# omkhairate/MetalPathtracer

Hardware: AMD Instinct MI355X
Metric: Mrays/s at 1920x1080x256spp on scene.xml (higher is better)
Workload: dtype f32; 1 GPU; scene.xml 1920x1080 x 256 spp per step, depth 8 (181 steps timed); prims=4971, bvh_nodes=2289, bvh_builder=device, rng=philox4x32-10 (pixel,sample,bounce), pipeline=wave-local wavefront, reference-order walk, parallelism=8x8-tile interleave over 1 rank(s), rays=161154900585

## Files before the change

metalpathtracer_amd/csrc/mpt_kernels.h:

```cpp
#pragma once
#include <hip/hip_runtime.h>
#include <stdint.h>

#include "mpt_device.h"
#include "mpt_wl_lean.h"
#include "mpt_lean_entry.h"
#include "mpt_lean_tiles.h"

#ifndef MPT_MIN_WAVES
#define MPT_MIN_WAVES 8
#endif

struct QueueDev {
    float4* od;
    float4* dt;
    float4* tl;
    uint2* ia;
};

struct PassDesc {
    uint32_t in_count[MPT_NSHARD];
    uint32_t item_prefix[MPT_NSHARD + 1];
    uint32_t n_items;
    uint32_t regen_base;
// ... 353 lines not shown
__device__ __forceinline__ void announce_resident(const PassParams& pp) {
    if (pp.launch_id == 0u) return;
    const uint32_t before = atomicAdd(&pp.ctr[MPT_CTR_STARTED], 1u);
    if (before == 0u) __hip_atomic_store(&pp.desc->t_first, (unsigned long long)__builtin_amdgcn_s_memrealtime(), __ATOMIC_RELAXED, __HIP_MEMORY_SCOPE_AGENT);
    if (before + 1u == gridDim.x)
        __hip_atomic_store((uint32_t*)pp.host_done + MPT_HOST_RESIDENT, pp.launch_id, __ATOMIC_RELAXED, __HIP_MEMORY_SCOPE_SYSTEM);
}

__device__ __forceinline__ void note_wave_exit(const PassParams& pp) {
    if (pp.launch_id == 0u || (threadIdx.x & 63u) != 0u) return;
    const uint32_t before = atomicAdd(&pp.ctr[MPT_CTR_EXITED], 1u);
    if (before + 1u == gridDim.x * (blockDim.x >> 6)) {
        const unsigned long long t0 = __hip_atomic_load(&pp.desc->t_first, __ATOMIC_RELAXED, __HIP_MEMORY_SCOPE_AGENT);
        atomicAdd(&pp.desc->trace_ticks, (unsigned long long)__builtin_amdgcn_s_memrealtime() - t0);
    }
}

__global__ void k_begin_pass(PassDesc* d, uint32_t* ctr, uint32_t total_paths, uint32_t slots_items,
                             volatile uint32_t* host_done, int path_cursors) {
    if (threadIdx.x != 0 || blockIdx.x != 0) return;
    ctr[MPT_CTR_STARTED] = 0u;
    ctr[MPT_CTR_EXITED] = 0u;
    if (path_cursors) {
        d->total_paths = total_paths;
        for (uint32_t g = 0; g < MPT_NGROUP; ++g) ctr[MPT_CTR_CURSOR(g)] = 0u;
        return;
    }
    for (uint32_t s = 0; s < MPT_NSHARD; ++s) ctr[MPT_CTR_OUT(s)] = 0;
    d->next_path = 0;
    d->total_paths = total_paths;
    d->slots_items = slots_items;
    d->iterations = 0;
    advance_desc(d, ctr, host_done);
}

__global__ void k_advance(PassDesc* d, uint32_t* ctr, volatile uint32_t* host_done) {
    if (threadIdx.x != 0 || blockIdx.x != 0) return;
    advance_desc(d, ctr, host_done);
}

template <bool COUNT, bool ALL_LDS>
__global__ __launch_bounds__(1024, MPT_MIN_WAVES) void k_megakernel(PassParams pp) {
    extern __shared__ float4 lds_nodes[];
    stage_nodes(pp.scene, lds_nodes);
    const uint32_t lane = threadIdx.x & 63u;
    const uint32_t total_paths = pp.desc->total_paths;
    const uint32_t waves_per_block = blockDim.x >> 6;
    uint32_t n_rays = 0, n_paths = 0;
    WorkCount wc = {};
    for (uint32_t chunk = blockIdx.x * waves_per_block + (threadIdx.x >> 6); chunk * 64u < total_paths;
         chunk += gridDim.x * waves_per_block) {
        PathState ps;
        PathRngDev g;
        ps.path = chunk * 64u + lane;
        uint32_t px, py, s;
        if (!path_to_pixel(pp, ps.path, px, py, s)) continue;
        gen_primary(pp, px, py, pp.sample_begin + s, ps, g);
        n_paths++;
        bool alive = true;
        while (alive) {
            float t;
            int prim;
            closest_hit<COUNT, ALL_LDS>(pp.scene, (LdsNodes)lds_nodes, ps.o, ps.d, t, prim, wc);
            n_rays++;
            alive = shade_bounce(pp.scene, (LdsNodes)lds_nodes, pp.sp, g, ps, t, prim);
        }
        pp.slots[ps.path] = make_float4(clamp01(ps.L.x), clamp01(ps.L.y), clamp01(ps.L.z), clamp01(ps.La));
    }
    flush_stats<COUNT>(pp.desc, n_rays, n_paths, wc);
}

typedef float v4f_nt __attribute__((ext_vector_type(4)));
__device__ __forceinline__ void store_slot(float4* slots, uint32_t path, float r, float g, float b, float a) {
    v4f_nt v = {r, g, b, a};
    __builtin_nontemporal_store(v, (v4f_nt*)(slots + path));
}
__device__ __forceinline__ float4 load_slot(const float4* slots, uint32_t idx) {
    v4f_nt v = __builtin_nontemporal_load((const v4f_nt*)(slots + idx));
    return make_float4(v.x, v.y, v.z, v.w);
}

__device__ __forceinline__ uint32_t wave_rank(unsigned long long m) {
    return __builtin_amdgcn_mbcnt_hi((uint32_t)(m >> 32), __builtin_amdgcn_mbcnt_lo((uint32_t)m, 0u));
}

#ifndef MPT_WL_LEVELS
#define MPT_WL_LEVELS 2u
#endif
#define MPT_WL_RING 512u
#define MPT_LDS_MATS_N 32u
#define MPT_LDS_CFG_F4 16u
static_assert(CFG_F4_END <= MPT_LDS_CFG_F4, "configuration block too small");
__host__ __device__ __forceinline__ uint32_t mpt_lds_cfg_off_f4(uint32_t lds_mat_off) { return lds_mat_off + 2u * MPT_LDS_MATS_N; }
__host__ __device__ __forceinline__ uint32_t mpt_lds_image_end_f4(uint32_t lds_mat_off) { return mpt_lds_cfg_off_f4(lds_mat_off) + MPT_LDS_CFG_F4; }
#define MPT_WL_BLOCK 1024u
#define MPT_WL_TILE_ELIDED 0x40000000u
static_assert((MPT_WL_TILE_ELIDED & (MPT_LEAN_TILES_SKIP | MPT_LEAN_TILES_MASK_BITS)) == 0u, "the elision mark shares a bit with the class word");
#define MPT_WL_NO_BUDGET 0x7FFFFFFFu

__device__ __forceinline__ void cfg_stage_common(float4* blk, const PassParams& pp, float rW, float rH, uint32_t wl_block, uint32_t wl_min, uint32_t wl_div) {
    blk[CFG_F4_CAM] = make_float4(pp.cam.x, pp.cam.y, pp.cam.z, pp.W);
    blk[CFG_F4_FIRST] = make_float4(pp.first.x, pp.first.y, pp.first.z, pp.H);
    blk[CFG_F4_VU] = make_float4(pp.vu.x, pp.vu.y, pp.vu.z, rW);
    blk[CFG_F4_VV] = make_float4(pp.vv.x, pp.vv.y, pp.vv.z, rH);
    uint32_t* w = (uint32_t*)(blk + CFG_F4_WORDS);
    w[CFG_W_CLAIM_BLOCK] = wl_block;
    w[CFG_W_CLAIM_MIN] = wl_min;
    w[CFG_W_CLAIM_DIV] = wl_div * (((uint32_t)(gridDim.x * (blockDim.x >> 6)) + MPT_NGROUP - 1u) / MPT_NGROUP);
    w[CFG_W_RANK_TILES] = pp.desc->total_paths / (pp.S * 64u);
}
__device__ __forceinline__ CamView cfg_cam_view(LdsNodes blk) {
    const v4f c0 = blk[CFG_F4_CAM], c1 = blk[CFG_F4_FIRST], c2 = blk[CFG_F4_VU], c3 = blk[CFG_F4_VV];
    CamView cv;
    cv.cam = f3(c0.x, c0.y, c0.z);
    cv.first = f3(c1.x, c1.y, c1.z);
    cv.vu = f3(c2.x, c2.y, c2.z);
    cv.vv = f3(c3.x, c3.y, c3.z);
    cv.W = c0.w;
    cv.H = c1.w;
    cv.rW = c2.w;
    cv.rH = c3.w;
    return cv;
}
__device__ __forceinline__ bool claim_paths(const PassParams& pp, LdsWords cfg, uint32_t lane, uint32_t& grp, uint32_t& seen, uint32_t& k, uint32_t& blk,
                                            uint32_t& rend) {
    bool got = false;
    k = 0, blk = 0, rend = 0;
    if (lane == 0) {
        const uint32_t c_block = cfg[CFG_W_CLAIM_BLOCK], c_min = cfg[CFG_W_CLAIM_MIN], c_div = cfg[CFG_W_CLAIM_DIV], c_tiles = cfg[CFG_W_RANK_TILES];
        for (uint32_t t = 0; t < MPT_NGROUP && !got; ++t) {
            const uint32_t re = range_paths(c_tiles, pp.S, grp);
            const uint32_t left = seen < re ? re - seen : 0u;
            blk = (left / c_div) & ~63u;
            blk = blk < c_min ? c_min : (blk > c_block ? c_block : blk);
            if (t > 0u) blk = c_min;
            k = atomicAdd(&pp.ctr[MPT_CTR_CURSOR(grp)], blk);
            if (k < re) {
                got = true;
                rend = re;
            } else {
                grp = (grp + 1u) & (MPT_NGROUP - 1u);
                seen = 0;
            }
        }
    }
    got = __builtin_amdgcn_readfirstlane((int)got) != 0;
    k = __builtin_amdgcn_readfirstlane(k);
    blk = __builtin_amdgcn_readfirstlane(blk);
    rend = __builtin_amdgcn_readfirstlane(rend);
    grp = __builtin_amdgcn_readfirstlane(grp);
    seen = k;
    return got;
}
#define MPT_RING_HAS_LIGHT 0x100u
struct WaveRings {
    float4* base;
    uint32_t n;
    __host__ __device__ float4* od() const { return base; }
    __host__ __device__ float4* dt() const { return base + n; }
    __host__ __device__ float4* tl() const { return base + 2u * (size_t)n; }
    __host__ __device__ uint4* ia() const { return (uint4*)(base + 3u * (size_t)n); }
    __host__ __device__ uint4* tv() const { return (uint4*)(base + 4u * (size_t)n); }
};
__device__ __forceinline__ bool ring_has_light(const PathState& ps) {
    return (__float_as_uint(ps.L.x) | __float_as_uint(ps.L.y) | __float_as_uint(ps.L.z) | __float_as_uint(ps.La)) != 0u;
}
__device__ __forceinline__ uint32_t sample_of_path(const PassParams& pp, uint32_t path) {
    const uint32_t chunk = path >> 6;
    return pp.sample_begin + (pp.s_shift != 0xFFu ? chunk & (pp.S - 1u) : chunk % pp.S);
}
__device__ __forceinline__ void ring_push(const WaveRings& ring, uint32_t at, const PathState& ps, const PathRngDev& g) {
    ring.od()[at] = make_float4(ps.o.x, ps.o.y, ps.o.z, ps.d.x);
    ring.dt()[at] = make_float4(ps.d.y, ps.d.z, ps.thr.x, ps.thr.y);
    const bool lit = ring_has_light(ps);
    ring.ia()[at] = make_uint4(__float_as_uint(ps.thr.z), ps.path, g.pixel, ps.bounce | (lit ? MPT_RING_HAS_LIGHT : 0u));
    if (lit) ring.tl()[at] = make_float4(ps.L.x, ps.L.y, ps.L.z, ps.La);
}
__device__ __forceinline__ void ring_pop(const PassParams& pp, const WaveRings& ring, uint32_t at, PathState& ps, PathRngDev& g) {
    const float4 a = ring.od()[at], b = ring.dt()[at];
    const uint4 ia = ring.ia()[at];
    ps.o = f3(a.x, a.y, a.z);
    ps.d = f3(a.w, b.x, b.y);
    ps.thr = f3(b.z, b.w, __uint_as_float(ia.x));
    ps.path = ia.y;
    g.pixel = ia.z;
    ps.bounce = ia.w & 0xFFu;
    g.sample = sample_of_path(pp, ps.path);
    ps.L = f3(0.0f, 0.0f, 0.0f);
    ps.La = 0.0f;
    if ((ia.w & MPT_RING_HAS_LIGHT) != 0u) {
        const float4 cc = ring.tl()[at];
        ps.L = f3(cc.x, cc.y, cc.z);
        ps.La = cc.w;
    }
    g.lit_seed = 0;
    if (pp.sp.rng_mode == 0) g.lit_seed = pcg_hash(pcg_hash(pp.pixel_seed[g.pixel]));
}
__device__ __forceinline__ void ring_push_hit(const WaveRings& ring, uint32_t at, const PathState& ps, float t, uint32_t prim) {
    ring.od()[at] = make_float4(ps.o.x, ps.o.y, ps.o.z, ps.d.x);
    ring.dt()[at] = make_float4(ps.d.y, ps.d.z, ps.thr.x, ps.thr.y);
    const bool lit = ring_has_light(ps);
    ring.ia()[at] = make_uint4(__float_as_uint(ps.thr.z), ps.path, (__float_as_uint(t) & 0x7FFFFFFFu) | (lit ? 0x80000000u : 0u),
                               (prim & 0x07FFFFFFu) | (ps.bounce << 27));
    if (lit) ring.tl()[at] = make_float4(ps.L.x, ps.L.y, ps.L.z, ps.La);
}
__device__ __forceinline__ void ring_pop_hit(const WaveRings& ring, uint32_t at, PathState& ps, float& t, int& prim) {
    const float4 a = ring.od()[at], b = ring.dt()[at];
    const uint4 ia = ring.ia()[at];
    ps.o = f3(a.x, a.y, a.z);
    ps.d = f3(a.w, b.x, b.y);
    ps.thr = f3(b.z, b.w, __uint_as_float(ia.x));
    ps.path = ia.y;
    t = __uint_as_float(ia.z & 0x7FFFFFFFu);
    prim = (int)(ia.w & 0x07FFFFFFu);
    ps.bounce = ia.w >> 27;
    ps.L = f3(0.0f, 0.0f, 0.0f);
    ps.La = 0.0f;
    if ((ia.z & 0x80000000u) != 0u) {
        const float4 cc = ring.tl()[at];
        ps.L = f3(cc.x, cc.y, cc.z);
        ps.La = cc.w;
    }
}

struct WaveBudgets {
    uint32_t b[MPT_WL_LEVELS];
    uint32_t min_active[MPT_WL_LEVELS];
};

#ifndef MPT_WL_THREADS_N
#define MPT_WL_THREADS_N 768
#endif
#ifndef MPT_WL_WAVES_N
#define MPT_WL_WAVES_N 6
#endif
#define MPT_WL_THREADS(ALL_LDS) MPT_WL_THREADS_N
#define MPT_WL_WAVES(ALL_LDS) MPT_WL_WAVES_N
template <bool COUNT, bool ALL_LDS, bool LEAN = false>
__device__ __forceinline__ void wavelocal_body(const PassParams& pp, const WaveRings& ring, const WaveBudgets& budgets, uint32_t wl_block, uint32_t wl_min,
                                               uint32_t wl_div, const WlLean& lean = WlLean{0u, 0u, 0u}, const uint32_t* tile_classes = nullptr,
                                               uint32_t sky_resolve = 0u);
template <bool COUNT, bool ALL_LDS>
__global__ __launch_bounds__(MPT_WL_THREADS(ALL_LDS), MPT_WL_WAVES(ALL_LDS)) void k_wavelocal(PassParams pp, WaveRings ring, WaveBudgets budgets,
                                                                                             uint32_t wl_block, uint32_t wl_min, uint32_t wl_div) {
    wavelocal_body<COUNT, ALL_LDS>(pp, ring, budgets, wl_block, wl_min, wl_div);
}
#ifndef MPT_WL_CORUN_SGPRS
#define MPT_WL_CORUN_SGPRS 96
#endif
template <bool ALL_LDS>
__global__ __launch_bounds__(MPT_WL_THREADS(ALL_LDS), MPT_WL_WAVES(ALL_LDS)) __attribute__((amdgpu_num_sgpr(MPT_WL_CORUN_SGPRS)))
void k_wavelocal_corun(PassParams pp, WaveRings ring, WaveBudgets budgets, uint32_t wl_block, uint32_t wl_min, uint32_t wl_div) {
    wavelocal_body<false, ALL_LDS>(pp, ring, budgets, wl_block, wl_min, wl_div);
}
template <bool ALL_LDS>
__global__ __launch_bounds__(MPT_WL_THREADS(ALL_LDS), MPT_WL_WAVES(ALL_LDS)) void k_wavelocal_lean(PassParams pp, WaveRings ring, WaveBudgets budgets,
                                                                                                  uint32_t wl_block, uint32_t wl_min, uint32_t wl_div, WlLean lean,
                                                                                                  const uint32_t* tile_classes, uint32_t sky_resolve) {
    wavelocal_body<false, ALL_LDS, true>(pp, ring, budgets, wl_block, wl_min, wl_div, lean, tile_classes, sky_resolve);
}
template <bool ALL_LDS>
__global__ __launch_bounds__(MPT_WL_THREADS(ALL_LDS), MPT_WL_WAVES(ALL_LDS)) __attribute__((amdgpu_num_sgpr(MPT_WL_CORUN_SGPRS)))
void k_wavelocal_lean_corun(PassParams pp, WaveRings ring, WaveBudgets budgets, uint32_t wl_block, uint32_t wl_min, uint32_t wl_div, WlLean lean,
                            const uint32_t* tile_classes, uint32_t sky_resolve) {
    wavelocal_body<false, ALL_LDS, true>(pp, ring, budgets, wl_block, wl_min, wl_div, lean, tile_classes, sky_resolve);
}
__global__ __launch_bounds__(64) void k_lean_tile_classes(const float4* nodes, uint32_t n_nodes, const float4* prims, uint32_t n_prims, LeanTileView view,
                                                          uint32_t* out, uint32_t n_words) {
    const uint32_t T = blockIdx.x * blockDim.x + threadIdx.x;
    if (T >= n_words) return;
    const uint32_t ty = T / view.tiles_x, tx = T - ty * view.tiles_x;
    out[T] = ty < view.tiles_y ? lean_tile_class(nodes, n_nodes, prims, n_prims, view, tx, ty) : 0u;
}
struct WaveStepDiag {
    enum Region { SELECT, FETCH, TRACE, SHADE, PUSH, N_REGIONS };
#ifdef MPT_DEBUG_WAVE_TIMES
    unsigned long long t_start, t_exh = 0ull, t_claim = 0ull, steps = 0ull, left = 0ull, blk = 0ull;
    unsigned long long reg[N_REGIONS] = {}, tic_;
    WorkCount wc0;
    __device__ __forceinline__ static uint32_t n_waves() { return gridDim.x * (blockDim.x >> 6); }
    __device__ __forceinline__ static unsigned long long* buffer(const WaveRings& ring) { return (unsigned long long*)(ring.tv() + (size_t)n_waves() * MPT_WL_LEVELS * MPT_WL_RING); }
    __device__ __forceinline__ void start() { t_start = __builtin_amdgcn_s_memrealtime(); }
    __device__ __forceinline__ void tic() { tic_ = __builtin_amdgcn_s_memtime(); }
    __device__ __forceinline__ void toc(Region r) { MPT_TOC(reg[r], tic_); }
    __device__ __forceinline__ void claimed(bool got, uint32_t asked, const uint32_t* cnt) {
        if (got) {
            t_claim = __builtin_amdgcn_s_memrealtime();
            steps = 0ull;
            blk = asked;
        } else {
            t_exh = __builtin_amdgcn_s_memrealtime();
            for (uint32_t q = 0; q < MPT_WL_LEVELS; ++q) left |= (unsigned long long)cnt[q] << (12u * q);
        }
    }
    __device__ __forceinline__ void step(bool exhausted, int level) {
        if (!exhausted) steps += 1ull << (12u * (uint32_t)(level + 1));
    }
    __device__ __forceinline__ void before_walk(const WorkCount& wc) { wc0 = wc; }
    template <bool COUNT>
    __device__ __forceinline__ void after_walk(const WaveRings& ring, int level, const WorkCount& wc, bool done) const {
        if (!COUNT) return;
        unsigned long long* lv = buffer(ring) + 16ull * n_waves() + 8ull * (unsigned)(level + 1);
        if (first_active_lane()) atomicAdd(lv + 0, 1ull);
        if (wc.node_iters != wc0.node_iters) atomicAdd(lv + 1, (unsigned long long)(wc.node_iters - wc0.node_iters));
        if (wc.prim_iters != wc0.prim_iters) atomicAdd(lv + 3, (unsigned long long)(wc.prim_iters - wc0.prim_iters));
        atomicAdd(lv + 2, (unsigned long long)(wc.node_visits - wc0.node_visits));
        atomicAdd(lv + 4, (unsigned long long)(wc.prim_tests - wc0.prim_tests));
        atomicAdd(lv + 5, 1ull);
        if (wc.wait_leaf != wc0.wait_leaf) atomicAdd(lv + 7, (unsigned long long)(wc.wait_leaf - wc0.wait_leaf));
        if (done) atomicAdd(lv + 6, 1ull);
        unsigned long long* lo = lv + 8ull * 8ull;
        for (int q = 0; q < 3; ++q) {
            const uint32_t n = wc.low_trips[q] - wc0.low_trips[q];
            if (n != 0u) atomicAdd(lo + q, (unsigned long long)n);
            if (__ballot(n != 0u) != 0ull && first_active_lane()) atomicAdd(lo + 3 + q, 1ull);
        }
    }
    template <bool COUNT>
    __device__ __forceinline__ void traffic(const WaveRings& ring, uint32_t lane, unsigned long long am, unsigned long long pm, bool keep, bool alive, bool parked,
                                            const PathState& ps) const {
        if (!COUNT || (am | pm) == 0ull) return;
        unsigned long long* rt = buffer(ring) + 16ull * n_waves() + 8ull * 14ull;
        const unsigned long long lit_a = __ballot(alive && ring_has_light(ps)), lit_p = __ballot(parked && ring_has_light(ps));
        if (lane == 0u) {
            if (am != 0ull) {
                atomicAdd(rt + 8 + (keep ? 0 : 1), (unsigned long long)__popcll(am));
                atomicAdd(rt + 8 + (keep ? 2 : 3), (unsigned long long)__popcll(lit_a));
                atomicAdd(rt + 8 + (keep ? 4 : 5), 1ull);
            }
            if (pm != 0ull) {
                atomicAdd(rt + 0, (unsigned long long)__popcll(pm));
                atomicAdd(rt + 1, (unsigned long long)__popcll(lit_p));
                atomicAdd(rt + 2, 1ull);
            }
        }
    }
    __device__ __forceinline__ void finish(const WaveRings& ring, uint32_t lane, uint32_t wave_id, const WorkCount& wc) const {
        if (lane != 0) return;
        unsigned long long* dbg = buffer(ring);
        dbg[8 * wave_id] = t_start;
        dbg[8 * wave_id + 1] = t_exh;
        dbg[8 * wave_id + 2] = __builtin_amdgcn_s_memrealtime();
        dbg[8 * wave_id + 3] = t_claim;
        dbg[8 * wave_id + 4] = steps;
        dbg[8 * wave_id + 5] = left;
        dbg[8 * wave_id + 6] = blk;
        unsigned long long* out = dbg + 8ull * n_waves() + 8ull * wave_id;
        for (int r = 0; r < N_REGIONS; ++r) out[r] = reg[r];
        out[5] = wc.t_box;
        out[6] = wc.t_leaf;
    }
#else
    __device__ __forceinline__ void start() {}
    __device__ __forceinline__ void tic() {}
    __device__ __forceinline__ void toc(Region) {}
    __device__ __forceinline__ void claimed(bool, uint32_t, const uint32_t*) {}
    __device__ __forceinline__ void step(bool, int) {}
    __device__ __forceinline__ void before_walk(const WorkCount&) {}
    template <bool COUNT>
    __device__ __forceinline__ void after_walk(const WaveRings&, int, const WorkCount&, bool) const {}
    template <bool COUNT>
    __device__ __forceinline__ void traffic(const WaveRings&, uint32_t, unsigned long long, unsigned long long, bool, bool, bool, const PathState&) const {}
    __device__ __forceinline__ void finish(const WaveRings&, uint32_t, uint32_t, const WorkCount&) const {}
#endif
};
template <bool ALL_LDS>
__device__ __forceinline__ void cfg_stage_lean(float4* blk, const PassParams& pp) {
    const float4 none = make_float4(0.0f, 0.0f, 0.0f, 0.0f);
    const bool tree = pp.scene.n_nodes != 0u;
    const LeanEntry e = lean_entry_terms(tree ? pp.scene.nodes[0] : none, tree ? pp.scene.nodes[1] : none, pp.scene.n_nodes, pp.cam.x, pp.cam.y, pp.cam.z);
    uint32_t entry = e.entry, entry_primary = e.entry_primary;
    if (ALL_LDS) {
        const LeanTail t = lean_tail_terms(pp.scene.nodes, pp.scene.n_nodes, pp.cam.x, pp.cam.y, pp.cam.z);
        float4* const tail = blk + CFG_F4_TAIL;
        tail[CFG_TAIL_LO] = make_float4(t.tlo[0], t.tlo[1], t.tlo[2], __uint_as_float(t.leaf));
        tail[CFG_TAIL_HI] = make_float4(t.thi[0], t.thi[1], t.thi[2], __uint_as_float(t.tail_primary));
        float4 t0 = make_float4(0.0f, 0.0f, 0.0f, 0.0f), t1 = t0;
        if (t.node != 0u) {
            t0 = pp.scene.nodes[2u * t.node];
            t1 = pp.scene.nodes[2u * t.node + 1u];
        }
        t1.w = __uint_as_float(t.node);
        tail[CFG_TAIL_N0] = t0;
        tail[CFG_TAIL_N1] = t1;
        if (t.node != 0u && entry == t.node) entry = MPT_NODE_TAIL;
        if (t.node != 0u && entry_primary == t.node) entry_primary = MPT_NODE_TAIL;
    }
    blk[CFG_F4_ENTRY_LO] = make_float4(e.ilo[0], e.ilo[1], e.ilo[2], __uint_as_float(entry));
    blk[CFG_F4_ENTRY_HI] = make_float4(e.ihi[0], e.ihi[1], e.ihi[2], __uint_as_float(entry_primary));
}
template <bool COUNT, bool ALL_LDS, bool LEAN>
__device__ __forceinline__ void wavelocal_body(const PassParams& pp, const WaveRings& ring, const WaveBudgets& budgets, uint32_t wl_block, uint32_t wl_min,
                                               uint32_t wl_div, const WlLean& lean, const uint32_t* tile_classes, uint32_t sky_resolve) {
    static_assert(!(LEAN && COUNT), "the lean body does not count");
    constexpr bool TILES = LEAN && ALL_LDS;
#if defined(MPT_LEAN_RING_TESTING)
    constexpr bool RING_CONSTS = false;
#else
    constexpr bool RING_CONSTS = LEAN && MPT_WL_LEVELS == 2u;
#endif
    extern __shared__ float4 lds_nodes_raw[];
    const uint32_t cfg_off = mpt_lds_cfg_off_f4(pp.scene.lds_mat_off);
    float4* const blk_raw = lds_nodes_raw + cfg_off;
    if (threadIdx.x == 0) {
        announce_resident(pp);
        cfg_stage_common(blk_raw, pp, LEAN ? cdiv_recip(pp.W) : 0.0f, LEAN ? cdiv_recip(pp.H) : 0.0f, wl_block, wl_min, wl_div);
        uint32_t* w = (uint32_t*)(blk_raw + CFG_F4_WORDS);
        static_assert(MPT_WL_LEVELS <= CFG_MAX_LEVELS, "configuration block: a budget word per ring");
        for (uint32_t k = 0; k < MPT_WL_LEVELS; ++k) {
            w[CFG_W_BUDGET + k] = budgets.b[k];
            w[CFG_W_MIN_ACTIVE + k] = budgets.min_active[k];
        }
        if (LEAN) {
            w[CFG_W_S_MUL] = lean.s_mul;
            w[CFG_W_S_SHIFT] = lean.s_shift;
        }
        if (TILES) {
            w[CFG_W_CLASSES_LO] = (uint32_t)(uintptr_t)tile_classes;
            w[CFG_W_CLASSES_HI] = (uint32_t)((uint64_t)(uintptr_t)tile_classes >> 32);
            static_assert(MPT_WL_LEVELS < CFG_MAX_LEVELS, "configuration block: CFG_W_SKY_RESOLVE lies in the last ring's minimum");
            w[CFG_W_SKY_RESOLVE] = tile_classes != nullptr ? sky_resolve : 0u;
        }
        if (LEAN) cfg_stage_lean<ALL_LDS>(blk_raw, pp);
    }
    if (LEAN) stage_nodes_lean(pp.scene, lds_nodes_raw, pp.cam);
    else stage_nodes(pp.scene, lds_nodes_raw);
    if (LEAN && ALL_LDS) {
        const uint32_t tail_node = __float_as_uint(blk_raw[CFG_F4_TAIL + CFG_TAIL_N1].w);
        if (tail_node != 0u) {
            uint32_t* links = (uint32_t*)lds_nodes_raw;
            for (uint32_t k = threadIdx.x; k < pp.scene.n_lds_nodes * 2u; k += blockDim.x)
                if (links[4u * k + 3u] == tail_node) links[4u * k + 3u] = MPT_NODE_TAIL;
        }
        __syncthreads();
    }
    MPT_CLOCK_BEGIN();
    const LdsNodes lds_nodes = (LdsNodes)lds_nodes_raw;
    const LdsNodes blk = lds_nodes + cfg_off;
    const LdsWords lds_cfg_u32 = (LdsWords)(blk + CFG_F4_WORDS);
    const uint32_t lane = threadIdx.x & 63u;
    const uint32_t wave_id = blockIdx.x * (blockDim.x >> 6) + (threadIdx.x >> 6);
    const uint32_t wbase = wave_id * (MPT_WL_LEVELS * MPT_WL_RING);
    const uint32_t M = MPT_WL_RING - 1u;
    uint32_t cnt[MPT_WL_LEVELS];
#pragma unroll
    for (uint32_t k = 0; k < MPT_WL_LEVELS; ++k) cnt[k] = 0;
    uint32_t cur = 0, end = 0;
    uint32_t grp = blockIdx.x & (MPT_NGROUP - 1u);
    uint32_t seen = 0;
    bool exhausted = false;
    uint32_t tile_cached = 0xFFFFFFFFu, tile_xy_cached = 0u;
    uint32_t tile_class_cached = 0u;
    float uvx_cached = 0.0f, uvy_cached = 0.0f;
    uint32_t n_rays = 0, n_paths = 0;
    WorkCount wc = {};
    bool kept = false;
    PathState ps = {};
    float best_t = INFINITY;
    int best_prim = -1;
    WaveStepDiag diag;
    diag.start();
    for (;;) {
        diag.tic();
        int level = -1;
        const unsigned long long carry = __ballot(kept);
        if (cnt[0] + (uint32_t)__popcll(carry) >= 64u) level = 0;
#pragma unroll
        for (int k = (int)MPT_WL_LEVELS - 1; k >= 1; --k)
            if (level <= 0 && cnt[k] >= 64u) level = k;
        if (level < 0) {
            if (!exhausted && cur == end) {
                uint32_t k, blk_asked, rend;
                const bool got = claim_paths(pp, lds_cfg_u32, lane, grp, seen, k, blk_asked, rend);
                diag.claimed(got, blk_asked, cnt);
                if (!got) {
                    exhausted = true;
                } else {
                    cur = k;
                    end = (k + blk_asked < rend) ? k + blk_asked : rend;
                }
            }
            if (exhausted) {
                uint32_t total = 0;
#pragma unroll
                for (int k = 0; k < (int)MPT_WL_LEVELS; ++k) total += cnt[k];
                if (total == 0u) break;
                level = (int)MPT_WL_LEVELS;
            }
        }
        diag.step(exhausted, level);
        diag.toc(WaveStepDiag::SELECT);
        float hit_t = __uint_as_float(__float_as_uint(best_t) & 0x7FFFFFFFu);
        int hit_prim = (int)((uint32_t)best_prim & 0x07FFFFFFu);
        ps.bounce &= 31u;
        best_t = INFINITY;
        best_prim = -1;
        PathRngDev g;
        bool valid = false;
        uint32_t node = 0;
        uint32_t budget = 0xFFFFFFFFu, min_active = 0u;
        bool fresh = false;
        bool need_shade = false;
        if (level < 0) {
            fresh = true;
            const uint32_t pchunk = range_chunk_to_path_chunk(pp, cur >> 6, grp);
            cur += 64u;
            uint32_t tl, sidx;
            chunk_tile_sample(pp, pchunk, tl, sidx);
            const bool new_tile = tl != tile_cached;
            if (new_tile) {
                tile_cached = tl;
                if (TILES) {
                    const uint32_t tlo = (uint32_t)__builtin_amdgcn_readfirstlane((int)lds_cfg_u32[CFG_W_CLASSES_LO]), thi = (uint32_t)__builtin_amdgcn_readfirstlane((int)lds_cfg_u32[CFG_W_CLASSES_HI]);
                    tile_class_cached = 0u;
                    if ((tlo | thi) != 0u) {
                        typedef const __attribute__((address_space(4))) uint32_t* ConstWords;
                        tile_class_cached = ((ConstWords)(((uint64_t)thi << 32) | tlo))[tl * pp.nranks + pp.rank];
                        if (tile_class_cached == MPT_LEAN_TILES_SKIP && (uint32_t)__builtin_amdgcn_readfirstlane((int)lds_cfg_u32[CFG_W_SKY_RESOLVE]) != 0u)
                            tile_class_cached = MPT_LEAN_TILES_SKIP | MPT_WL_TILE_ELIDED;
                    }
                }
                if (TILES) {
                } else if (LEAN) {
                    const uint32_t T = tl * pp.nranks + pp.rank, ty = (T * lean.tile_mul) >> MPT_WL_LEAN_TILE_SHIFT;
                    tile_xy_cached = (T - ty * pp.tiles_x) | (ty << 16);
                } else {
                    tile_xy_cached = (uint32_t)__builtin_amdgcn_readfirstlane((int)pp.tile_xy[tl]);
                }
            }
            PathState np;
            np.path = pchunk * 64u + lane;
            uint32_t tile_xy = tile_xy_cached;
            if (TILES) {
                const uint32_t T = tl * pp.nranks + pp.rank, ty = (T * lean.tile_mul) >> MPT_WL_LEAN_TILE_SHIFT;
                tile_xy = (T - ty * pp.tiles_x) | (ty << 16);
            }
            const uint32_t px = (tile_xy & 0xFFFFu) * 8u + (lane & 7u), py = (tile_xy >> 16) * 8u + (lane >> 3);
            if (TILES && (tile_class_cached & MPT_WL_TILE_ELIDED) != 0u) {
                const uint32_t left = (end - cur) >> 6, more = pp.S - 1u - sidx < left ? pp.S - 1u - sidx : left;
                const uint32_t elided = (uint32_t)__popcll(__ballot(px < pp.width && py < pp.height)) * (1u + more);
                cur += more * 64u;
                n_paths += elided;
                n_rays += elided;
                continue;
            }
            const CamView cv = cfg_cam_view(blk);
            if (new_tile) pixel_uv(cv, px, py, uvx_cached, uvy_cached);
            if (px < pp.width && py < pp.height) {
                gen_primary<LEAN>(pp, cv, px, py, uvx_cached, uvy_cached, pp.sample_begin + sidx, np, g);
                valid = true;
            }
            n_paths += (uint32_t)__popcll(__ballot(valid));
            ps = np;
        } else {
            uint32_t my_ring = 0, my_off = 0;
            bool take = false;
            uint32_t assigned = 0;
            const uint32_t slot = wave_rank(~carry), room = 64u - (uint32_t)__popcll(carry);
            const bool empty = !kept;
#pragma unroll
            for (int k = (int)MPT_WL_LEVELS - 1; k >= 0; --k) {
                const bool use = (level == (int)MPT_WL_LEVELS) || (level == k);
                uint32_t tk = use ? cnt[k] : 0u;
                tk = tk < room - assigned ? tk : room - assigned;
                if (empty && slot >= assigned && slot < assigned + tk) {
                    take = true;
                    my_ring = (uint32_t)k;
                    my_off = cnt[k] - tk + (slot - assigned);
                }
                cnt[k] -= tk;
                assigned += tk;
            }
            if (RING_CONSTS) {
                if (level < (int)MPT_WL_LEVELS) {
                    budget = level == 0 ? MPT_LEAN_RING0_BUDGET : MPT_WL_NO_BUDGET;
                    min_active = level == 0 ? MPT_LEAN_RING0_N0 : MPT_LEAN_RING1_N;
                }
            } else if (level < (int)MPT_WL_LEVELS) {
                budget = (uint32_t)__builtin_amdgcn_readfirstlane((int)lds_cfg_u32[CFG_W_BUDGET + level]);
                min_active = (uint32_t)__builtin_amdgcn_readfirstlane((int)lds_cfg_u32[CFG_W_MIN_ACTIVE + level]);
            }
            if (level == (int)MPT_WL_LEVELS && assigned >= 12u) min_active = assigned / 3u;
            if (take) {
                const uint32_t at = wbase + my_ring * MPT_WL_RING + my_off;
                uint4 tv = make_uint4(0u, 0u, 0u, 0u);
                if (my_ring > 0u) tv = ring.tv()[at];
                ring_pop_hit(ring, at, ps, hit_t, hit_prim);
                need_shade = my_ring == 0u;
                if (my_ring > 0u) {
                    node = tv.x;
                    best_t = __uint_as_float(tv.y);
                    best_prim = (int)tv.z;
                } else {
                    fresh = true;
                }
                valid = true;
            }
            if (kept) {
                need_shade = true;
                fresh = true;
                valid = true;
            }
        }
        if (need_shade) {
            uint32_t px, py, sidx;
            path_to_pixel<LEAN>(pp, ps.path, px, py, sidx, lean.tile_mul, lds_cfg_u32);
            g.pixel = LEAN ? mul_u24(py, pp.width) + px : py * pp.width + px;
            g.sample = pp.sample_begin + sidx;
            g.lit_seed = 0;
            if (!LEAN && pp.sp.rng_mode == 0) g.lit_seed = pcg_hash(pcg_hash(pp.pixel_seed[g.pixel]));
            if (!shade_bounce<LEAN>(pp.scene, lds_nodes, pp.sp, g, ps, hit_t, hit_prim)) {
                store_slot(pp.slots, ps.path, clamp01(ps.L.x), clamp01(ps.L.y), clamp01(ps.L.z), clamp01(ps.La));
                valid = false;
            }
        }
        if (LEAN && fresh) {
            const bool d_ok = fmaxf(fmaxf(fabsf(ps.d.x), fabsf(ps.d.y)), fabsf(ps.d.z)) <= MPT_LEAN_ENTRY_DMAX;
            if (level < 0) {
                const uint32_t entry_primary = ((LdsWords)(blk + CFG_F4_ENTRY_HI))[CFG_W_OF_F4];
                node = d_ok ? entry_primary : 0u;
            } else {
                const v4f elo = blk[CFG_F4_ENTRY_LO], ehi = blk[CFG_F4_ENTRY_HI];
                const bool in = elo.x <= ps.o.x && ps.o.x <= ehi.x && elo.y <= ps.o.y && ps.o.y <= ehi.y && elo.z <= ps.o.z && ps.o.z <= ehi.z;
                node = in && d_ok ? __float_as_uint(elo.w) : 0u;
            }
        }
        const bool budgeted = level >= 0 && (level < (int)MPT_WL_LEVELS || min_active != 0u) &&
                              ((level < (int)MPT_WL_LEVELS - 1 && budget < MPT_WL_NO_BUDGET) || min_active != 0u);
        const int park_ring = level + 1 < (int)MPT_WL_LEVELS ? level + 1 : (int)MPT_WL_LEVELS - 1;
        bool alive = false, parked = false;
        diag.toc(WaveStepDiag::FETCH);
        diag.before_walk(wc);
        n_rays += (uint32_t)__popcll(__ballot(valid && fresh));
        if (valid) {
            bool done;
            if (budgeted)
                done = closest_hit_resume<COUNT, ALL_LDS, true, LEAN>(pp.scene, lds_nodes, ps.o, ps.d, node, best_t, best_prim,
                                                                     budget, wc, min_active, blk + CFG_F4_TAIL);
            else if (LEAN && level < 0)
                done = closest_hit_resume<COUNT, ALL_LDS, false, LEAN, true>(pp.scene, lds_nodes, ps.o, ps.d, node, best_t, best_prim,
                                                                            0xFFFFFFFFu, wc, 0u, blk + CFG_F4_TAIL, TILES ? tile_class_cached : 0u);
            else
                done = closest_hit_resume<COUNT, ALL_LDS, false, LEAN>(pp.scene, lds_nodes, ps.o, ps.d, node, best_t, best_prim,
                                                                      0xFFFFFFFFu, wc, 0u, blk + CFG_F4_TAIL);
            diag.toc(WaveStepDiag::TRACE);
            diag.template after_walk<COUNT>(ring, level, wc, done);
            if (done) {
                alive = best_prim >= 0;
                if (!alive) {
                    shade_bounce<LEAN>(pp.scene, lds_nodes, pp.sp, g, ps, best_t, -1);
                    store_slot(pp.slots, ps.path, clamp01(ps.L.x), clamp01(ps.L.y), clamp01(ps.L.z), clamp01(ps.La));
                }
            } else {
                parked = true;
            }
        }
        diag.toc(WaveStepDiag::SHADE);
        const unsigned long long am = __ballot(alive), pm = __ballot(parked);
        if (pm != 0ull) {
            uint32_t c = 0;
#pragma unroll
            for (int k = 1; k < (int)MPT_WL_LEVELS; ++k)
                if (k == park_ring) c = cnt[k];
            if (parked) {
                const uint32_t at = wbase + (uint32_t)park_ring * MPT_WL_RING + ((c + wave_rank(pm)) & M);
                ring_push_hit(ring, at, ps, 0.0f, 0u);
                ring.tv()[at] = make_uint4(node, __float_as_uint(best_t), (uint32_t)best_prim, 0u);
            }
#pragma unroll
            for (int k = 1; k < (int)MPT_WL_LEVELS; ++k)
                if (k == park_ring) cnt[k] = c + (uint32_t)__popcll(pm);
        }
        bool keep = cnt[0] + (uint32_t)__popcll(am) >= 64u;
#pragma unroll
        for (int k = 1; k < (int)MPT_WL_LEVELS; ++k) keep = keep && cnt[k] < 64u;
        kept = keep && alive;
        diag.template traffic<COUNT>(ring, lane, am, pm, keep, alive, parked, ps);
        if (am != 0ull && !keep) {
            if (alive) {
                const uint32_t at = wbase + ((cnt[0] + wave_rank(am)) & M);
                ring_push_hit(ring, at, ps, best_t, (uint32_t)best_prim);
            }
            cnt[0] += (uint32_t)__popcll(am);
        }
        uint32_t worst = 0;
#pragma unroll
        for (uint32_t k = 0; k < MPT_WL_LEVELS; ++k) worst = cnt[k] > worst ? cnt[k] : worst;
        if (worst > MPT_WL_RING) pp.desc->overflow = 1u;
        diag.toc(WaveStepDiag::PUSH);
    }
    diag.finish(ring, lane, wave_id, wc);
    MPT_CLOCK_END();
    flush_stats<COUNT>(pp.desc, lane == 0u ? n_rays : 0u, lane == 0u ? n_paths : 0u, wc);
    note_wave_exit(pp);
}

#ifndef MPT_RESOLVE_SGPRS
#define MPT_RESOLVE_SGPRS 56
#endif
__device__ __forceinline__ CamView resolve_cam_view(const PassParams& pp) {
    return CamView{pp.cam, pp.first, pp.vu, pp.vv, pp.W, pp.H, cdiv_recip(pp.W), cdiv_recip(pp.H)};
}
__device__ __forceinline__ bool resolve_sky_tile(const PassParams& pp, const uint32_t* sky_classes, uint32_t tl) {
    if (sky_classes == nullptr) return false;
    const uint32_t T = (uint32_t)__builtin_amdgcn_readfirstlane((int)tl) * pp.nranks + pp.rank;
    return sky_classes[T] == MPT_LEAN_TILES_SKIP;
}
#if defined(MPT_SKY_RESOLVE_CONTROL) && !defined(MPT_SKY_RESOLVE_TESTING)
#error "MPT_SKY_RESOLVE_CONTROL makes the resolve's sky samples wrong on purpose: test builds only (-DMPT_SKY_RESOLVE_TESTING)"
#endif
__device__ __forceinline__ float4 resolve_sky_sample(const PassParams& pp, const CamView& cv, uint32_t px, uint32_t py, float uvx, float uvy, uint32_t s) {
    PathState ps;
    PathRngDev g;
#if defined(MPT_SKY_RESOLVE_CONTROL)
    s += 1u;
#endif
    gen_primary<true>(pp, cv, px, py, uvx, uvy, pp.sample_begin + s, ps, g);
    shade_bounce<true>(pp.scene, (LdsNodes)nullptr, pp.sp, g, ps, INFINITY, -1);
    return make_float4(clamp01(ps.L.x), clamp01(ps.L.y), clamp01(ps.L.z), clamp01(ps.La));
}
__device__ __forceinline__ void add_sample(float4& acc, const float4& v) {
    acc.x += v.x; acc.y += v.y; acc.z += v.z; acc.w += v.w;
}
__global__ __launch_bounds__(256, 8) __attribute__((amdgpu_num_sgpr(MPT_RESOLVE_SGPRS))) void k_resolve_sum(PassParams pp, float4* sum, uint32_t n_local_tiles, const uint32_t* sky_classes) {
    const uint32_t n = n_local_tiles * 64u;
    for (uint32_t i = blockIdx.x * blockDim.x + threadIdx.x; i < n; i += gridDim.x * blockDim.x) {
        const uint32_t tl = i >> 6, lane = i & 63u;
        const bool sky = resolve_sky_tile(pp, sky_classes, tl);
        uint32_t px, py, s0;
        if (!path_to_pixel(pp, (tl * pp.S) * 64u + lane, px, py, s0)) continue;
        float4 acc = sum[py * pp.width + px];
        const uint32_t base = tl * pp.S;
        uint32_t s = 0;
        if (sky) {
            const CamView cv = resolve_cam_view(pp);
            float uvx, uvy;
            pixel_uv(cv, px, py, uvx, uvy);
            for (; s + 2u <= pp.S; s += 2u) {
                const float4 v0 = resolve_sky_sample(pp, cv, px, py, uvx, uvy, s), v1 = resolve_sky_sample(pp, cv, px, py, uvx, uvy, s + 1u);
                add_sample(acc, v0);
                add_sample(acc, v1);
            }
            if (s < pp.S) add_sample(acc, resolve_sky_sample(pp, cv, px, py, uvx, uvy, s));
            sum[py * pp.width + px] = acc;
            continue;
        }
        for (; s + 4u <= pp.S; s += 4u) {
            const float4 v0 = load_slot(pp.slots, (base + s) * 64u + lane), v1 = load_slot(pp.slots, (base + s + 1u) * 64u + lane),
                         v2 = load_slot(pp.slots, (base + s + 2u) * 64u + lane), v3 = load_slot(pp.slots, (base + s + 3u) * 64u + lane);
            add_sample(acc, v0);
            add_sample(acc, v1);
            add_sample(acc, v2);
            add_sample(acc, v3);
        }
        for (; s < pp.S; ++s) add_sample(acc, load_slot(pp.slots, (base + s) * 64u + lane));
        sum[py * pp.width + px] = acc;
    }
}

__device__ __forceinline__ void add_moments(float4& m, const float4& v) {
    const float l = (0.2126f * v.x + 0.7152f * v.y) + 0.0722f * v.z;
    m.x += v.x * v.x; m.y += v.y * v.y; m.z += v.z * v.z; m.w += l * l;
}
__global__ __launch_bounds__(256, 8) __attribute__((amdgpu_num_sgpr(MPT_RESOLVE_SGPRS))) void k_resolve_sum_moments(PassParams pp, float4* sum, float4* m2, uint32_t n_local_tiles, const uint32_t* sky_classes) {
    const uint32_t n = n_local_tiles * 64u;
    for (uint32_t i = blockIdx.x * blockDim.x + threadIdx.x; i < n; i += gridDim.x * blockDim.x) {
        const uint32_t tl = i >> 6, lane = i & 63u;
        const bool sky = resolve_sky_tile(pp, sky_classes, tl);
        uint32_t px, py, s0;
        if (!path_to_pixel(pp, (tl * pp.S) * 64u + lane, px, py, s0)) continue;
        float4 acc = sum[py * pp.width + px];
        float4 m = m2[py * pp.width + px];
        const uint32_t base = tl * pp.S;
        uint32_t s = 0;
        if (sky) {
            const CamView cv = resolve_cam_view(pp);
            float uvx, uvy;
            pixel_uv(cv, px, py, uvx, uvy);
            for (; s + 2u <= pp.S; s += 2u) {
                const float4 v0 = resolve_sky_sample(pp, cv, px, py, uvx, uvy, s), v1 = resolve_sky_sample(pp, cv, px, py, uvx, uvy, s + 1u);
                add_sample(acc, v0);
                add_sample(acc, v1);
                add_moments(m, v0);
                add_moments(m, v1);
            }
            if (s < pp.S) {
                const float4 v = resolve_sky_sample(pp, cv, px, py, uvx, uvy, s);
                add_sample(acc, v);
                add_moments(m, v);
            }
            sum[py * pp.width + px] = acc;
            m2[py * pp.width + px] = m;
            continue;
        }
        for (; s + 4u <= pp.S; s += 4u) {
            const float4 v0 = load_slot(pp.slots, (base + s) * 64u + lane), v1 = load_slot(pp.slots, (base + s + 1u) * 64u + lane),
                         v2 = load_slot(pp.slots, (base + s + 2u) * 64u + lane), v3 = load_slot(pp.slots, (base + s + 3u) * 64u + lane);
            add_sample(acc, v0);
            add_sample(acc, v1);
            add_sample(acc, v2);
            add_sample(acc, v3);
            add_moments(m, v0);
            add_moments(m, v1);
            add_moments(m, v2);
            add_moments(m, v3);
        }
        for (; s < pp.S; ++s) {
            const float4 v = load_slot(pp.slots, (base + s) * 64u + lane);
            add_sample(acc, v);
            add_moments(m, v);
        }
// ... 118 lines not shown
```

Before: 76090 Mrays/s.

## Prefetch next path-block claim, add straight-line fast path for fully-alive waves

In the lean kernel, the next work-block atomic claim is issued as soon as a claim is consumed, so the atomic's latency overlaps primary-ray generation instead of stalling the select step; work stealing falls back to fixed-size claims from other groups. A straight path is added for two-level rings: when every lane carried a live path and ring 1 has room, the wave skips level selection, the ring fetch and the push and continues bouncing in registers. The budgeted-walk test is simplified so all non-primary levels go through the budgeted walk. Debug counters for claim wait and head statistics are added. The costs are extra live registers for the pending claim and a change to how rings are scheduled, which could affect occupancy or load balance.

```diff
diff --git a/metalpathtracer_amd/csrc/mpt_kernels.h b/metalpathtracer_amd/csrc/mpt_kernels.h
--- a/metalpathtracer_amd/csrc/mpt_kernels.h
+++ b/metalpathtracer_amd/csrc/mpt_kernels.h
@@ -529,6 +529,53 @@
     seen = k;
     return got;
 }
+#if defined(MPT_CLAIM_AHEAD_CONTROL) && !defined(MPT_CLAIM_AHEAD_TESTING)
+#error "MPT_CLAIM_AHEAD_CONTROL drops claimed path ids on purpose: test builds only (-DMPT_CLAIM_AHEAD_TESTING)"
+#endif
+__device__ __forceinline__ uint32_t claim_ahead_issue(const PassParams& pp, LdsWords cfg, uint32_t lane, uint32_t grp, uint32_t seen) {
+    const uint32_t c_block = cfg[CFG_W_CLAIM_BLOCK], c_min = cfg[CFG_W_CLAIM_MIN], c_div = cfg[CFG_W_CLAIM_DIV], c_tiles = cfg[CFG_W_RANK_TILES];
+    const uint32_t re = range_paths(c_tiles, pp.S, grp);
+    const uint32_t left = seen < re ? re - seen : 0u;
+    uint32_t blk = (left / c_div) & ~63u;
+    blk = blk < c_min ? c_min : (blk > c_block ? c_block : blk);
+    uint32_t pend = lane == 1u ? blk : re;
+    uint32_t zero;
+    asm("v_mov_b32 %0, 0" : "=v"(zero));
+    if (lane == 0) pend = atomicAdd(&pp.ctr[MPT_CTR_CURSOR(grp) + zero], blk);
+    return pend;
+}
+__device__ __forceinline__ bool claim_ahead_take(uint32_t pend, uint32_t& k, uint32_t& blk, uint32_t& rend) {
+    k = (uint32_t)__builtin_amdgcn_readlane((int)pend, 0);
+    blk = (uint32_t)__builtin_amdgcn_readlane((int)pend, 1);
+    rend = (uint32_t)__builtin_amdgcn_readlane((int)pend, 2);
+#if defined(MPT_CLAIM_AHEAD_CONTROL)
+    if (k + blk >= rend) return false;
+#endif
+    return k < rend;
+}
+__device__ __forceinline__ bool claim_steal(const PassParams& pp, LdsWords cfg, uint32_t lane, uint32_t& grp, uint32_t& k, uint32_t& blk, uint32_t& rend) {
+    bool got = false;
+    k = 0, blk = 0, rend = 0;
+    if (lane == 0) {
+        const uint32_t c_min = cfg[CFG_W_CLAIM_MIN], c_tiles = cfg[CFG_W_RANK_TILES];
+        for (uint32_t t = 1; t < MPT_NGROUP && !got; ++t) {
+            grp = (grp + 1u) & (MPT_NGROUP - 1u);
+            const uint32_t re = range_paths(c_tiles, pp.S, grp);
+            blk = c_min;
+            k = atomicAdd(&pp.ctr[MPT_CTR_CURSOR(grp)], blk);
+            if (k < re) {
+                got = true;
+                rend = re;
+            }
+        }
+    }
+    got = __builtin_amdgcn_readfirstlane((int)got) != 0;
+    k = __builtin_amdgcn_readfirstlane(k);
+    blk = __builtin_amdgcn_readfirstlane(blk);
+    rend = __builtin_amdgcn_readfirstlane(rend);
+    grp = __builtin_amdgcn_readfirstlane(grp);
+    return got;
+}
 #define MPT_RING_HAS_LIGHT 0x100u
 struct WaveRings {
     float4* base;
@@ -660,7 +707,16 @@
     __device__ __forceinline__ void start() { t_start = __builtin_amdgcn_s_memrealtime(); }
     __device__ __forceinline__ void tic() { tic_ = __builtin_amdgcn_s_memtime(); }
     __device__ __forceinline__ void toc(Region r) { MPT_TOC(reg[r], tic_); }
+    unsigned long long claim_wait = 0ull, heads = 0ull, claim_tic_;
+    bool new_claim = false;
+    __device__ __forceinline__ void claim_tic() { claim_tic_ = __builtin_amdgcn_s_memtime(); }
+    __device__ __forceinline__ void claim_toc() { MPT_TOC(claim_wait, claim_tic_); }
+    __device__ __forceinline__ void first_tile(bool elided) {
+        if (new_claim) heads += elided ? 1ull << 16 : 1ull;
+        new_claim = false;
+    }
     __device__ __forceinline__ void claimed(bool got, uint32_t asked, const uint32_t* cnt) {
+        new_claim = got;
         if (got) {
             t_claim = __builtin_amdgcn_s_memrealtime();
             steps = 0ull;
@@ -670,8 +726,9 @@
             for (uint32_t q = 0; q < MPT_WL_LEVELS; ++q) left |= (unsigned long long)cnt[q] << (12u * q);
         }
     }
-    __device__ __forceinline__ void step(bool exhausted, int level) {
+    __device__ __forceinline__ void step(bool exhausted, int level, bool all_carried) {
         if (!exhausted) steps += 1ull << (12u * (uint32_t)(level + 1));
+        if (!exhausted && level == 0) heads += (1ull << 48) + (all_carried ? 1ull << 32 : 0ull);
     }
     __device__ __forceinline__ void before_walk(const WorkCount& wc) { wc0 = wc; }
     template <bool COUNT>
@@ -722,17 +779,22 @@
         dbg[8 * wave_id + 4] = steps;
         dbg[8 * wave_id + 5] = left;
         dbg[8 * wave_id + 6] = blk;
+        dbg[8 * wave_id + 7] = claim_wait;
         unsigned long long* out = dbg + 8ull * n_waves() + 8ull * wave_id;
         for (int r = 0; r < N_REGIONS; ++r) out[r] = reg[r];
         out[5] = wc.t_box;
         out[6] = wc.t_leaf;
+        out[7] = heads;
     }
 #else
     __device__ __forceinline__ void start() {}
     __device__ __forceinline__ void tic() {}
     __device__ __forceinline__ void toc(Region) {}
+    __device__ __forceinline__ void claim_tic() {}
+    __device__ __forceinline__ void claim_toc() {}
     __device__ __forceinline__ void claimed(bool, uint32_t, const uint32_t*) {}
-    __device__ __forceinline__ void step(bool, int) {}
+    __device__ __forceinline__ void first_tile(bool) {}
+    __device__ __forceinline__ void step(bool, int, bool) {}
     __device__ __forceinline__ void before_walk(const WorkCount&) {}
     template <bool COUNT>
     __device__ __forceinline__ void after_walk(const WaveRings&, int, const WorkCount&, bool) const {}
@@ -771,6 +833,8 @@
                                                uint32_t wl_div, const WlLean& lean, const uint32_t* tile_classes, uint32_t sky_resolve) {
     static_assert(!(LEAN && COUNT), "the lean body does not count");
     constexpr bool TILES = LEAN && ALL_LDS;
+    constexpr bool AHEAD = LEAN, TWO_WALKS = LEAN;
+    constexpr bool STRAIGHT = LEAN && MPT_WL_LEVELS == 2u;
 #if defined(MPT_LEAN_RING_TESTING)
     constexpr bool RING_CONSTS = false;
 #else
@@ -826,6 +890,8 @@
     uint32_t grp = blockIdx.x & (MPT_NGROUP - 1u);
     uint32_t seen = 0;
     bool exhausted = false;
+    uint32_t pend = 0;
+    if (AHEAD) pend = claim_ahead_issue(pp, lds_cfg_u32, lane, grp, 0u);
     uint32_t tile_cached = 0xFFFFFFFFu, tile_xy_cached = 0u;
     uint32_t tile_class_cached = 0u;
     float uvx_cached = 0.0f, uvy_cached = 0.0f;
@@ -841,20 +907,32 @@
         diag.tic();
         int level = -1;
         const unsigned long long carry = __ballot(kept);
-        if (cnt[0] + (uint32_t)__popcll(carry) >= 64u) level = 0;
+        const bool straight = STRAIGHT && carry == ~0ull;
+        if (straight) level = 0;
+        if (!straight && cnt[0] + (uint32_t)__popcll(carry) >= 64u) level = 0;
 #pragma unroll
         for (int k = (int)MPT_WL_LEVELS - 1; k >= 1; --k)
-            if (level <= 0 && cnt[k] >= 64u) level = k;
+            if (!straight && level <= 0 && cnt[k] >= 64u) level = k;
+        bool claim_new = false;
         if (level < 0) {
             if (!exhausted && cur == end) {
                 uint32_t k, blk_asked, rend;
-                const bool got = claim_paths(pp, lds_cfg_u32, lane, grp, seen, k, blk_asked, rend);
+                bool got;
+                diag.claim_tic();
+                if (AHEAD) {
+                    got = claim_ahead_take(pend, k, blk_asked, rend);
+                    if (!got) got = claim_steal(pp, lds_cfg_u32, lane, grp, k, blk_asked, rend);
+                } else {
+                    got = claim_paths(pp, lds_cfg_u32, lane, grp, seen, k, blk_asked, rend);
+                }
+                diag.claim_toc();
                 diag.claimed(got, blk_asked, cnt);
                 if (!got) {
                     exhausted = true;
                 } else {
                     cur = k;
                     end = (k + blk_asked < rend) ? k + blk_asked : rend;
+                    claim_new = true;
                 }
             }
             if (exhausted) {
@@ -865,7 +943,7 @@
                 level = (int)MPT_WL_LEVELS;
             }
         }
-        diag.step(exhausted, level);
+        diag.step(exhausted, level, carry == ~0ull);
         diag.toc(WaveStepDiag::SELECT);
         float hit_t = __uint_as_float(__float_as_uint(best_t) & 0x7FFFFFFFu);
         int hit_prim = (int)((uint32_t)best_prim & 0x07FFFFFFu);
@@ -913,7 +991,9 @@
                 tile_xy = (T - ty * pp.tiles_x) | (ty << 16);
             }
             const uint32_t px = (tile_xy & 0xFFFFu) * 8u + (lane & 7u), py = (tile_xy >> 16) * 8u + (lane >> 3);
+            diag.first_tile(TILES && (tile_class_cached & MPT_WL_TILE_ELIDED) != 0u);
             if (TILES && (tile_class_cached & MPT_WL_TILE_ELIDED) != 0u) {
+                if (AHEAD && claim_new) pend = claim_ahead_issue(pp, lds_cfg_u32, lane, grp, cur - 64u);
                 const uint32_t left = (end - cur) >> 6, more = pp.S - 1u - sidx < left ? pp.S - 1u - sidx : left;
                 const uint32_t elided = (uint32_t)__popcll(__ballot(px < pp.width && py < pp.height)) * (1u + more);
                 cur += more * 64u;
@@ -922,6 +1002,7 @@
                 continue;
             }
             const CamView cv = cfg_cam_view(blk);
+            if (AHEAD && claim_new) pend = claim_ahead_issue(pp, lds_cfg_u32, lane, grp, cur - 64u);
             if (new_tile) pixel_uv(cv, px, py, uvx_cached, uvy_cached);
             if (px < pp.width && py < pp.height) {
                 gen_primary<LEAN>(pp, cv, px, py, uvx_cached, uvy_cached, pp.sample_begin + sidx, np, g);
@@ -929,6 +1010,15 @@
             }
             n_paths += (uint32_t)__popcll(__ballot(valid));
             ps = np;
+        } else if (straight) {
+            if (RING_CONSTS) {
+                budget = MPT_LEAN_RING0_BUDGET;
+                min_active = MPT_LEAN_RING0_N0;
+            } else {
+                budget = (uint32_t)__builtin_amdgcn_readfirstlane((int)lds_cfg_u32[CFG_W_BUDGET]);
+                min_active = (uint32_t)__builtin_amdgcn_readfirstlane((int)lds_cfg_u32[CFG_W_MIN_ACTIVE]);
+            }
+            need_shade = fresh = valid = true;
         } else {
             uint32_t my_ring = 0, my_off = 0;
             bool take = false;
@@ -1002,8 +1092,9 @@
                 node = in && d_ok ? __float_as_uint(elo.w) : 0u;
             }
         }
-        const bool budgeted = level >= 0 && (level < (int)MPT_WL_LEVELS || min_active != 0u) &&
-                              ((level < (int)MPT_WL_LEVELS - 1 && budget < MPT_WL_NO_BUDGET) || min_active != 0u);
+        const bool budgeted = TWO_WALKS ? level >= 0
+                                        : level >= 0 && (level < (int)MPT_WL_LEVELS || min_active != 0u) &&
+                                              ((level < (int)MPT_WL_LEVELS - 1 && budget < MPT_WL_NO_BUDGET) || min_active != 0u);
         const int park_ring = level + 1 < (int)MPT_WL_LEVELS ? level + 1 : (int)MPT_WL_LEVELS - 1;
         bool alive = false, parked = false;
         diag.toc(WaveStepDiag::FETCH);
@@ -1034,6 +1125,12 @@
         }
         diag.toc(WaveStepDiag::SHADE);
         const unsigned long long am = __ballot(alive), pm = __ballot(parked);
+        if (STRAIGHT && am == ~0ull && cnt[1] < 64u) {
+            kept = true;
+            diag.template traffic<COUNT>(ring, lane, am, 0ull, true, true, false, ps);
+            diag.toc(WaveStepDiag::PUSH);
+            continue;
+        }
         if (pm != 0ull) {
             uint32_t c = 0;
 #pragma unroll
```

Result: no change. 76750 Mrays/s, median of 6 (+0.9%).
